# nv-tlabs/brushstroke_engine

Hardware: AMD Instinct MI355X
Metric: stylized 256x256 stroke patches/sec at batch=32 (higher is better)
Workload: dtype f16 hi x f16 hi MFMA + 2 block-scaled fp8 (e4m3) correction products per fp32 product

## Files before the change

brushstroke_engine_amd/csrc/nb_modconv_h3.hip:

```cpp
#include "nb_h3_common.h"
#include "nb_torgb.h"

static int nb_noise_src_setup(const float* noise, int64_t stride_n, int ho, int wo, const float** k_noise, long long* k_stride, NbNoiseSrcDev* k_src) {
    *k_src = NbNoiseSrcDev{nullptr, nullptr, nullptr, nullptr, nullptr, 0, 0};
    if (stride_n != NB_NOISE_IN_KERNEL) { *k_noise = noise; *k_stride = stride_n; return NB_OK; }
    const NbNoiseSrc* s = reinterpret_cast<const NbNoiseSrc*>(noise);
    if (!s || !s->noise_const_t || !s->noise_lin || !s->noise_strength || ((s->norm_pos != nullptr) == (s->positions != nullptr))) return NB_EINVAL;
    if (s->res != ho || s->res != wo || (s->positions && s->img_resolution < 2)) return NB_EINVAL;
    *k_src = NbNoiseSrcDev{s->noise_const_t, s->noise_lin, s->noise_strength, s->norm_pos, (const long long*)s->positions, s->res, s->img_resolution};
    *k_noise = nullptr; *k_stride = 0;
    return NB_OK;
}

struct H3Params {
    const _Float16* x;
    const _Float16* wts;
    const float* dcoefs;
    const float* noise;
    NbNoiseSrcDev nsrc;
    const float* bias;
    float* y;
    const float* zeros;
    long long noise_stride_n;
    int c8, nchunks, c_out, co_ld, h, w;
// ... 1741 lines not shown
                        }
                    }
                unsigned ha[2][2], hb[2][2], la[2][2], lb[2][2];
#pragma unroll
                for (int px = 0; px < 2; ++px)
#pragma unroll
                    for (int k = 0; k < 2; ++k) {
                        ha[px][k] = hi[0][px][k]; hb[px][k] = hi[1][px][k]; la[px][k] = lo[0][px][k]; lb[px][k] = lo[1][px][k];
                        nb_swap32(ha[px][k], hb[px][k]);
                        nb_swap32(la[px][k], lb[px][k]);
                    }
                const int cg = co0 / 8 + 2 * R + gs;
                const int oy = 2 * qi + lh, ox = 2 * qj;
                if (qi < H && cg * 8 < p.c_out && !(p.dbg & 1)) {
                    const size_t OHW8 = (size_t)Ho * Wo * 8;
                    _Float16* yn = p.yh2 + ((size_t)n * p.c8_next + cg) * 2 * OHW8;
                    const size_t opix8 = ((size_t)oy * Wo + ox) * 8;
#pragma unroll
                    for (int px = 0; px < 2; ++px) {
                        *reinterpret_cast<u32x4*>(yn + opix8 + px * 8) = u32x4{ha[px][0], ha[px][1], hb[px][0], hb[px][1]};
                        if constexpr (OUTM == 1) {
                            *reinterpret_cast<u32x4*>(yn + OHW8 + opix8 + px * 8) = u32x4{la[px][0], la[px][1], lb[px][0], lb[px][1]};
                        } else {
                            _Float16* lo_xl = p.yh2 + ((size_t)n * p.c8_next + (cg & ~1)) * 2 * OHW8 + OHW8 + opix8 + px * 8 + (cg & 1) * 4;
                            *reinterpret_cast<u32x2*>(lo_xl) = u32x2{la[px][0], lb[px][0]};
                            *reinterpret_cast<u32x2*>(lo_xl + 2 * OHW8) = u32x2{la[px][1], lb[px][1]};
                        }
                    }
                }
            }
        };
        constexpr int NWI = nquads * 2 / 32;
        static_assert(nquads * 2 % 32 == 0, "tile quads must fill whole waves");
        if constexpr (NWI % NW == 0) {
#pragma unroll
            for (int k = 0; k < NWI / NW; ++k) quad_item(wv + k * NW);
        } else {
            for (int wi = wv; wi < NWI; wi += NW) quad_item(wi);
        }
        if (p.tstamps) { const unsigned long long t_ = __builtin_amdgcn_s_memtime(); te_f += t_ - te0; }
    }
    const unsigned long long te_s = 0;
    NB_TSTAMP(4);
    if (p.tstamps) {
        asm volatile("s_waitcnt vmcnt(0)" ::: "memory");
        NB_TSTAMP(5);
        if (threadIdx.x == 0) p.tstamps[(size_t)(blockIdx.x + blockIdx.y * gridDim.x) * 8 + 3] = (te_w & 0x1fffff) | ((te_f & 0x1fffff) << 21) | ((te_s & 0x1fffff) << 42);
    }
}

static int g_force_tqh = -1;
extern "C" void nb_debug_set_up2_tile(int tqh) { g_force_tqh = tqh; }
bool nb_up2v_eligible(int in_fmt, int c_in, int h, int w);
int nb_up2v_launch(H3Up2Params p, int n, int in_fmt, void* stream, unsigned long long* tstamps, int tstamps_cap);
#ifndef NB_UP2V_AUTO
#define NB_UP2V_AUTO 1
#endif
static int g_force_v2 = -1;
extern "C" void nb_debug_set_up2_v2(int mode) { g_force_v2 = mode; }
static int g_force_pair = -1;
extern "C" void nb_debug_set_up2_pair(int mode) { g_force_pair = mode; }
template <int TQH, int TQW, bool F8, int OUTM, int NW, int NST>
static int nb_up2_h3_launch1(const H3Up2Params& p, int n, size_t lds, void* stream) {
    static bool attr_set = false;
    if (!attr_set) {
        (void)hipFuncSetAttribute((const void*)modconv3x3_up2_h3_kernel<F8, TQH, OUTM, TQW, NW, NST>, hipFuncAttributeMaxDynamicSharedMemorySize, (int)lds);
        attr_set = true;
    }
    dim3 grid(p.tiles_x * p.tiles_y * p.slices, n);
    hipLaunchKernelGGL((modconv3x3_up2_h3_kernel<F8, TQH, OUTM, TQW, NW, NST>), grid, dim3(NW * 64), lds, (hipStream_t)stream, p);
    NB_CHECK_LAUNCH("modconv3x3_up2_h3");
    return NB_OK;
}

template <int TQH, int TQW = 32, int NW = 8, int NST = NB_H3_STAGES>
static int nb_up2_h3_launch(H3Up2Params p, int n, int in_fmt, void* stream) {
    p.tiles_x = p.w / TQW;
    p.tiles_y = (p.h + TQH - 1) / TQH;
    p.tstamps = (g_tstamps && (long long)p.tiles_x * p.tiles_y * p.slices * n <= g_tstamps_cap) ? g_tstamps : nullptr;
    constexpr int XPL = (TQH + 3) * (TQW + 3);
    constexpr int NBLK_ = ((TQH + 2) * (TQW + 2) + 31) / 32;
    constexpr size_t lds_stage = (size_t)NST * (4 * XPL + 36 * 32) * 16;
    static_assert(NBLK_ <= 2 * NW, "two column blocks per wave at most");
    constexpr size_t lds_epi = (size_t)16 * NBLK_ * 32 * 16;
    const size_t lds = lds_stage > lds_epi ? lds_stage : lds_epi;
    const int outm = p.yh2 ? (p.out_f8 ? 2 : 1) : 0;
    if constexpr (NW == 4) {
        NB_REQUIRE(!in_fmt, "modconv3x3_up2_h3: the two-workgroups-per-CU form takes H2 operands only");
        return outm == 2 ? nb_up2_h3_launch1<TQH, TQW, false, 2, NW, NST>(p, n, lds, stream) : outm == 1 ? nb_up2_h3_launch1<TQH, TQW, false, 1, NW, NST>(p, n, lds, stream)
                                                                                               : nb_up2_h3_launch1<TQH, TQW, false, 0, NW, NST>(p, n, lds, stream);
    } else
    if (in_fmt)
        return outm == 2 ? nb_up2_h3_launch1<TQH, TQW, true, 2, NW, NST>(p, n, lds, stream) : outm == 1 ? nb_up2_h3_launch1<TQH, TQW, true, 1, NW, NST>(p, n, lds, stream)
                                                                                              : nb_up2_h3_launch1<TQH, TQW, true, 0, NW, NST>(p, n, lds, stream);
    return outm == 2 ? nb_up2_h3_launch1<TQH, TQW, false, 2, NW, NST>(p, n, lds, stream) : outm == 1 ? nb_up2_h3_launch1<TQH, TQW, false, 1, NW, NST>(p, n, lds, stream)
                                                                                           : nb_up2_h3_launch1<TQH, TQW, false, 0, NW, NST>(p, n, lds, stream);
}

enum Up2Form { UP2_BIG = 0, UP2_MID, UP2_SMALL, UP2_W16, UP2_PAIR, UP2_WIDE, UP2_V2, UP2_W8 };
static Up2Form nb_up2_h3_select(int in_fmt, int c_in, int c_out, int n, int h, int w) {
    const int tiles_x = w / 32, slices = (c_out + 31) / 32;
    if (w == 16) return UP2_W16;
    if (w == 8) return UP2_W8;
    const int force_tqh = g_force_tqh >= 0 ? g_force_tqh : 0;
    const long wgs_big = (long)n * tiles_x * ((h + NB_H3_TQH - 1) / NB_H3_TQH) * slices;
    const bool small_tiles = force_tqh ? force_tqh == NB_H3_TQH_SMALL : wgs_big < 160;
    bool mid_tiles = force_tqh == NB_H3_TQH_MID;
    if (!force_tqh && !small_tiles) {
        constexpr long ncu = 256;
        const long wgs_mid = (long)n * tiles_x * ((h + NB_H3_TQH_MID - 1) / NB_H3_TQH_MID) * slices;
        const double est_big = (double)((wgs_big + ncu - 1) / ncu) * 5.4, est_mid = (double)((wgs_mid + ncu - 1) / ncu) * 3.93;
        mid_tiles = est_mid < 0.9 * est_big;
    }
    const bool pair = !in_fmt && g_force_pair > 0;
    if (pair) return UP2_PAIR;
    const int force_v2 = g_force_v2;
    if (force_v2 != 0 && nb_up2v_eligible(in_fmt, c_in, h, w) &&
        (force_v2 > 0 ? force_tqh == 0 || force_tqh == NB_H3_TQH : (NB_UP2V_AUTO && !mid_tiles && !small_tiles && (force_tqh == 0 || force_tqh == NB_H3_TQH))))
        return UP2_V2;
    if (mid_tiles) return UP2_MID;
    return small_tiles ? UP2_SMALL : UP2_BIG;
}

static int nb_up2_h3_impl(const void* x_h2, int c_in, const void* w_h3, const float* dcoefs, const float* noise,
                          int64_t noise_stride_n, const float* bias, float* y, void* y_h2, const float* next_styles,
                          int next_stride, int c_next, int n, int h, int w, int c_out, float alpha, float gain, float clamp,
                          void* stream, int in_fmt = 0, int out_fmt = 0) {
    NB_REQUIRE(in_fmt >= 0 && in_fmt <= 3 && (out_fmt == 0 || out_fmt == 1), "modconv3x3_up2_h3: input operand format must be 0 (H2), 1 (f8), 2 (f6) or 3 (f8, hi only), "
               "output format 0 or 1 (the up=2 epilogue does not write the f6 format)");
    NB_REQUIRE(in_fmt == 0 || c_in % 16 == 0, "modconv3x3_up2_h3: the f8 / f6 operand formats need c_in %% 16 == 0 (got %d)", c_in);
    NB_REQUIRE(out_fmt == 0 || (y_h2 && c_out % 16 == 0 && c_next % 16 == 0), "modconv3x3_up2_h3: f8 output needs an H2 destination and c_out, c_next %% 16 == 0");
    NB_REQUIRE(x_h2 && w_h3 && dcoefs && bias && ((y != nullptr) != (y_h2 != nullptr)), "modconv3x3_up2_h3: null pointer");
    NB_REQUIRE(!y_h2 || (next_styles && c_out % 8 == 0 && c_next >= c_out && next_stride >= c_out && (uintptr_t)y_h2 % 16 == 0),
               "modconv3x3_up2_h3: H2 output needs the consumer's styles, c_out %% 8 == 0 and c_next >= c_out");
    NB_REQUIRE(n > 0 && n <= 65535 && c_in > 0 && c_out > 0, "modconv3x3_up2_h3: bad sizes");
    NB_REQUIRE((w % 32 == 0 || w == 16 || w == 8) && h >= 8, "modconv3x3_up2_h3: needs w %% 32 == 0, w == 16 or w == 8 (got %dx%d)", h, w);
    NB_REQUIRE(alpha >= 0.f && alpha <= 1.f && gain > 0.f, "modconv3x3_up2_h3: leaky-ReLU slope must lie in [0, 1] and the gain be positive (got %g, %g)", alpha, gain);
    NB_REQUIRE(((uintptr_t)x_h2 | (uintptr_t)w_h3 | (uintptr_t)y) % 16 == 0, "modconv3x3_up2_h3: pointers must be 16-byte aligned");
    H3Up2Params p;
    p.x = (const _Float16*)x_h2; p.wts = (const _Float16*)w_h3; p.dcoefs = dcoefs; p.noise = noise; p.bias = bias; p.y = y;
    p.zeros = nb_zero_page_ptr();
    NB_REQUIRE(p.zeros, "modconv3x3_up2_h3: could not allocate the zero page");
    p.noise_stride_n = noise_stride_n;
    NB_REQUIRE(nb_noise_src_setup(noise, noise_stride_n, 2 * h, 2 * w, &p.noise, &p.noise_stride_n, &p.nsrc) == NB_OK, "modconv3x3_up2_h3: bad NbNoiseSrc (needs the "
               "transposed constant, the grid row, the strength, exactly one of norm_pos / positions, and res = the %dx%d output)", 2 * h, 2 * w);
    p.c8 = (c_in + 7) / 8; p.nchunks = (c_in + 15) / 16; p.c_out = c_out; p.co_ld = (c_out + 63) / 64 * 64; p.h = h; p.w = w;
    p.dbg = g_nb_debug_flags; p.stagger_ticks = g_nb_stagger_ticks;
    p.alpha = alpha; p.gain = gain; p.clamp = clamp;
    p.tiles_x = w / 32; p.slices = (c_out + 31) / 32;
    p.yh2 = (_Float16*)y_h2; p.next_styles = next_styles; p.next_stride = next_stride; p.c8_next = (c_next + 7) / 8;
    p.out_f8 = out_fmt;
    const Up2Form form = nb_up2_h3_select(in_fmt, c_in, c_out, n, h, w);
    NB_REQUIRE(in_fmt != 2 || form == UP2_V2, "modconv3x3_up2_h3: f6 operands are taken by the 12-row software-pipelined kernel only (this launch: %dx%d, batch %d)", h, w, n);
    switch (form) {
        case UP2_W16: return nb_up2_h3_launch<8, 16>(p, n, in_fmt, stream);
        case UP2_W8: return nb_up2_h3_launch<8, 8>(p, n, in_fmt, stream);
        case UP2_PAIR: return nb_up2_h3_launch<NB_H3_TQH, 16, 4, 2>(p, n, in_fmt, stream);
        case UP2_V2: return nb_up2v_launch(p, n, in_fmt, stream, g_tstamps, g_tstamps_cap);
        case UP2_MID: return nb_up2_h3_launch<NB_H3_TQH_MID>(p, n, in_fmt, stream);
        case UP2_SMALL: return nb_up2_h3_launch<NB_H3_TQH_SMALL>(p, n, in_fmt, stream);
        default: return nb_up2_h3_launch<NB_H3_TQH>(p, n, in_fmt, stream);
    }
}

extern "C" int nb_modconv3x3_up2_h3_variant(int in_fmt, int c_in, int c_out, int n, int h, int w, char* buf, int buflen) {
    NB_REQUIRE(buf && buflen > 0, "modconv3x3_up2_h3_variant: bad buffer");
    NB_REQUIRE(in_fmt >= 0 && in_fmt <= 3 && n > 0 && c_in > 0 && c_out > 0 && h >= 8 && (w % 32 == 0 || w == 16 || w == 8), "modconv3x3_up2_h3_variant: bad shape");
    static const char* const names[] = {"modconv3x3_up2_h3_kernel", "modconv3x3_up2_h3_kernel", "modconv3x3_up2_h3_kernel", "modconv3x3_up2_h3_kernel",
                                        "modconv3x3_up2_h3_kernel", "modconv3x3_up2_h3_kernel", "modconv3x3_up2v_kernel", "modconv3x3_up2_h3_kernel"};
    snprintf(buf, buflen, "%s", names[nb_up2_h3_select(in_fmt, c_in, c_out, n, h, w)]);
    return NB_OK;
}

extern "C" int nb_modconv3x3_up2_h3(const void* x_h2, int c_in, const void* w_h3, const float* dcoefs, const float* noise,
                                    int64_t noise_stride_n, const float* bias, float* y, int n, int h, int w, int c_out,
                                    float alpha, float gain, float clamp, void* stream) {
    return nb_up2_h3_impl(x_h2, c_in, w_h3, dcoefs, noise, noise_stride_n, bias, y, nullptr, nullptr, 0, 0, n, h, w, c_out,
                          alpha, gain, clamp, stream);
}

extern "C" int nb_modconv3x3_up2_h3_ex(const void* x, int c_in, const void* wts, const float* dcoefs, const float* noise,
                                      int64_t noise_stride_n, const float* bias, float* y_f32, void* y_h2,
                                      const float* next_styles, int next_stride, int c_next, int in_fmt, int out_fmt, int n,
                                      int h, int w, int c_out, float alpha, float gain, float clamp, void* stream) {
    return nb_up2_h3_impl(x, c_in, wts, dcoefs, noise, noise_stride_n, bias, y_f32, y_h2, next_styles, next_stride, c_next,
                          n, h, w, c_out, alpha, gain, clamp, stream, in_fmt, out_fmt);
}

extern "C" int nb_modconv3x3_up2_h3_h2(const void* x_h2, int c_in, const void* w_h3, const float* dcoefs, const float* noise,
                                       int64_t noise_stride_n, const float* bias, const float* next_styles, int next_stride,
                                       void* y_h2, int c_next, int n, int h, int w, int c_out, float alpha, float gain,
                                       float clamp, void* stream) {
    return nb_up2_h3_impl(x_h2, c_in, w_h3, dcoefs, noise, noise_stride_n, bias, nullptr, y_h2, next_styles, next_stride,
                          c_next, n, h, w, c_out, alpha, gain, clamp, stream);
}

__global__ __launch_bounds__(256) void pack_h2_kernel(const float* __restrict__ x1, int c1, const float* __restrict__ x2, int c2,
                                                      const float* __restrict__ scale, _Float16* __restrict__ out, int c8, int hw) {
    const int n = blockIdx.z, cg = blockIdx.y;
    const int pix = blockIdx.x * 256 + threadIdx.x;
    if (pix >= hw) return;
    const int c_in = c1 + c2;
    h8 hi, lo;
#pragma unroll
    for (int j = 0; j < 8; ++j) {
        const int ch = cg * 8 + j;
        float v = 0.f;
        if (ch < c_in) {
            v = ch < c1 ? x1[((size_t)n * c1 + ch) * hw + pix] : x2[((size_t)n * c2 + (ch - c1)) * hw + pix];
            if (scale) v *= scale[(size_t)n * c_in + ch];
        }
// ... 244 lines not shown
```

brushstroke_engine_amd/csrc/nb_modconv_up2v.hip:

```cpp
#include "nb_h3_common.h"

#ifdef NB_ABL6_NOMFMA
#define NB_ABL6_F16 false
#define NB_ABL6_FP6 false
#elif defined(NB_ABL6_NOFP6)
#define NB_ABL6_F16 true
#define NB_ABL6_FP6 false
#else
#define NB_ABL6_F16 true
#define NB_ABL6_FP6 true
#endif
#ifdef NB_ABL6_NODMA
#define NB_ABL_NODMA 1
#endif
namespace {
constexpr int TQH = 12, TQW = 32, NW = 8, NT = NW * 64;
constexpr int PH = TQH + 2, PW = TQW + 2, NPOS = PH * PW;
constexpr int NBLK = (NPOS + 31) / 32, NBJ = 2;
constexpr int XR = TQH + 3, XS = TQW + 3, XPL = XR * XS;
constexpr int PP = (XPL + 63) / 64, NXP = 4 * PP;
constexpr int CO_WG = 32, WROWS = 36, WSLOTS = WROWS * CO_WG, NWP = WSLOTS / 64;
constexpr int NPC = (NXP + NWP + NW - 1) / NW;
constexpr int STAGE = 4 * XPL + WSLOTS, NST = 3;
constexpr int N4 = 2;
constexpr int KMIX = NXP / NW;
static_assert(NBLK <= NBJ * NW && KMIX * NW <= NXP && (KMIX + 1) * NW > NXP && NPC == 7, "piece list layout");
}

template <bool F8, int OUTM, bool F6 = false, bool HO = false, bool PERSIST = true>
__global__ __launch_bounds__(NT, 2) void modconv3x3_up2v_kernel(const H3Up2Params p) {
    static_assert(!F6 || F8, "the f6 form is a variant of the f8 loop");
    static_assert(!HO || (F8 && !F6), "the hi-only form is a variant of the f8 loop");
    NB_TSTAMP(0);
    if constexpr (OUTM == 2) nb_set_fp16_ovfl();
    extern __shared__ __attribute__((aligned(16))) unsigned char smem_v[];
    h8* ring = reinterpret_cast<h8*>(smem_v);

    const int tid = threadIdx.x;
    const int lane = tid & 63, wv = __builtin_amdgcn_readfirstlane(tid >> 6), lh = lane >> 5, l31 = lane & 31;
    const int H = p.h, W = p.w;
    typedef const __attribute__((address_space(4))) H3Up2Params* kparams_t;
    auto fresh_params = [&]() -> kparams_t {
        kparams_t q = (kparams_t)__builtin_amdgcn_kernarg_segment_ptr();
        asm volatile("" : "+s"(q));
        return q;
    };
    const unsigned total = (unsigned)p.items;
    int n = 0, I0 = 0, J0 = 0, co0 = 0;
    const size_t HW8 = (size_t)H * W * 8;
    auto tile_coords = [&](unsigned l) {
        kparams_t q_ = fresh_params();
        const unsigned total = (unsigned)q_->items, gx = (unsigned)q_->items_x;
        const int dbg = q_->dbg, slices = q_->slices, tiles_x = q_->tiles_x;
        unsigned b = l % gx;
        unsigned nn = l / gx;
        if (total % 8 == 0 && gridDim.x % 8 == 0 && !(dbg & (8 | 32))) {
            const unsigned q = (l & 7) * (total >> 3) + (l >> 3);
            nn = q / gx; b = q - nn * gx;
        } else if (gx % 8 == 0 && !(dbg & 8)) b = (((b & 7) + nn) & 7) * (gx >> 3) + (b >> 3);
        const int slice = b % slices; b /= slices;
        const int tile_x = b % tiles_x; const int tile_y = b / tiles_x;
        n = __builtin_amdgcn_readfirstlane((int)nn); I0 = __builtin_amdgcn_readfirstlane(tile_y * TQH);
        J0 = __builtin_amdgcn_readfirstlane(tile_x * TQW); co0 = __builtin_amdgcn_readfirstlane(slice * CO_WG);
    };
    unsigned item = __builtin_amdgcn_readfirstlane(blockIdx.x);
    tile_coords(item);
    const int nblk = wv < NBLK - (NBJ - 1) * NW ? NBJ : NBJ - 1;

    __shared__ __attribute__((aligned(16))) float s_dco[CO_WG], s_bias[CO_WG], s_nst[CO_WG];
    __shared__ __attribute__((aligned(16))) float s_noise[2 * TQH * 2 * TQW];
    auto load_channel_tables = [&]() {
        kparams_t q_ = fresh_params();
        if (tid < CO_WG) {
            const int co = co0 + tid, c_out = q_->c_out;
            const float gain = q_->gain;
            s_dco[tid] = co < c_out ? q_->dcoefs[(size_t)n * c_out + co] * gain : 0.f;
            s_bias[tid] = co < c_out ? q_->bias[co] * gain : 0.f;
            s_nst[tid] = (q_->yh2 && co < c_out) ? q_->next_styles[(size_t)n * q_->next_stride + co] : 0.f;
        }
    };
    const unsigned lds0 = (unsigned)(uintptr_t)NB_LDS_PTR(smem_v);
    const size_t wchunk = (size_t)WROWS * p.co_ld * 16;
    const char* xsrc0[KMIX];
    unsigned xstr[KMIX];
    unsigned woff[NPC - KMIX - 1];
    const char* msrc0 = nullptr;
    unsigned mstr = 0;
    int xdst_s[KMIX + 1];
    unsigned xlast_bits = 0;
#pragma unroll
    for (int k = 0; k <= KMIX; ++k) {
        int q = k * NW + wv; q = q < NXP ? q : NXP - 1;
        const int pl = q / PP, part = q - pl * PP;
        xdst_s[k] = __builtin_amdgcn_readfirstlane(pl * XPL + part * 64);
        xlast_bits |= (part == PP - 1 ? 1u : 0u) << k;
    }
    xlast_bits = __builtin_amdgcn_readfirstlane(xlast_bits);
    auto xdst = [&](int k) { return xdst_s[k]; };
    auto xmask = [&](int k) -> unsigned long long { return (xlast_bits >> k) & 1u ? (1ull << (XPL - (PP - 1) * 64)) - 1 : ~0ull; };
    auto wq = [&](int k) { int q = k * NW + wv - NXP; return __builtin_amdgcn_readfirstlane(q < 0 ? 0 : (q < NWP ? q : NWP - 1)); };
    const bool mix_isx = KMIX * NW + wv < NXP;
    const int mdst = mix_isx ? xdst(KMIX) : 4 * XPL + wq(KMIX) * 64;
    const unsigned long long mmask = mix_isx ? xmask(KMIX) : ~0ull;
    auto piece_sources = [&]() {
        kparams_t q_ = fresh_params();
        const char* zeros = reinterpret_cast<const char*>(q_->zeros);
        const int co_ld = q_->co_ld;
        const _Float16* xn = q_->x + (size_t)n * q_->c8 * 2 * HW8;
        int i0_ = I0, j0_ = J0, c0_ = co0, lane_ = lane;
        asm volatile("" : "+v"(i0_), "+v"(j0_), "+v"(c0_), "+v"(lane_));
        i0_ = __builtin_amdgcn_readfirstlane(i0_); j0_ = __builtin_amdgcn_readfirstlane(j0_); c0_ = __builtin_amdgcn_readfirstlane(c0_);
        const char* xs_mix = zeros;
        unsigned xt_mix = 0, wo_mix = 0;
#pragma unroll
        for (int k = 0; k <= KMIX; ++k) {
            int q = k * NW + wv;
            q = q < NXP ? q : NXP - 1;
            const int pl = q / PP, part = q - pl * PP;
            const int e = part * 64 + lane_;
            const char* xs_ = zeros;
            unsigned xt_ = 0;
            if (e < XPL) {
                const int r = e / XS, c = e - r * XS;
// ... 342 lines not shown
        });
        if constexpr (MODE >= 2) asm volatile("s_waitcnt vmcnt(%0) lgkmcnt(0)\n\ts_barrier" ::"n"(NPC) : "memory");
        else if constexpr (MODE == 1) asm volatile("s_waitcnt vmcnt(0) lgkmcnt(0)\n\ts_barrier" ::: "memory");
        NB_FENCE();
        group_pair(std::integral_constant<int, 0>{}, ah_n, al_n, bh2, bh3, bl23, [&](auto g_) {
            constexpr int g = decltype(g_)::value;
            if constexpr (g == 2) dma(std::integral_constant<int, 0>{});
            if constexpr (g == 5) dma(std::integral_constant<int, 1>{});
            if constexpr (MODE >= 1) {
                if constexpr (g == 0) { ah_a[0] = rA(8, 0, san); rBh(bh0, J0_{}, 0, san); }
                else if constexpr (g == 1) { ah_a[1] = rA(6, 0, san); rBh(bh1, J0_{}, 1, san); }
                else if constexpr (g == 2) { rBh(bh0, J1_{}, 0, san); rBh(bh1, J1_{}, 1, san); }
                else if constexpr (g == 3) { set_lo(al_a, rA(8, 1, san)); set_hi(al_a, rA(6, 1, san)); }
                else if constexpr (g == 4) { rBl(bl01, 0, J0_{}, 0, san); rBl(bl01, 1, J0_{}, 1, san); }
                else { rBl(bl01, 0, J1_{}, 0, san); rBl(bl01, 1, J1_{}, 1, san); }
            }
        });
        NB_FENCE();
    };
    auto kloop = [&](auto nbe) {
        constexpr int NBE = decltype(nbe)::value;
        ah_a[0] = ring[aoff + 8 * 128]; ah_a[1] = ring[aoff + 6 * 128];
        if constexpr (F6) {
            const h8* b_ = ring + a6 + (lh ? 6 : 8) * 128;
            const i32x4 q0 = __builtin_bit_cast(i32x4, b_[0]); const i32x4 q1 = __builtin_bit_cast(i32x4, b_[64]);
            al6_a = v6i{q0[0], q0[1], q0[2], q0[3], q1[0], q1[1]}; sa6_a = q1[2];
        } else if constexpr (F8) { set_lo(al_a, ring[aoff + 8 * 128 + 32]); set_hi(al_a, ring[aoff + 6 * 128 + 32]); }
        else { hl_a[0] = ring[aoff + 8 * 128 + 32]; hl_a[1] = ring[aoff + 6 * 128 + 32]; }
#pragma unroll
        for (int j = 0; j < NBE; ++j) {
            bh0[j] = ring[boff[j]]; bh1[j] = ring[boff[j] + 1];
            if constexpr (F6) {
                const h8* b_ = ring + b6[j] + lh;
                const i32x4 q0 = __builtin_bit_cast(i32x4, b_[0]); const i32x4 q1 = __builtin_bit_cast(i32x4, b_[2 * XPL]);
                bl6_01[j] = v6i{q0[0], q0[1], q0[2], q0[3], q1[0], q1[1]}; sb6_01[j] = q1[2];
            } else if constexpr (F8) { set_lo(bl01[j], ring[boff[j] + XPL]); set_hi(bl01[j], ring[boff[j] + XPL + 1]); }
            else { bl0[j] = ring[boff[j] + XPL]; bl1[j] = ring[boff[j] + XPL + 1]; }
        }
        int c = 0, s = 0;
        auto nxt = [](int s_) { return s_ == 2 ? 0 : s_ + 1; };
        for (; c + 3 < NC; ++c) {
            chunk(std::integral_constant<int, 3>{}, nbe, c, ring + s * STAGE, ring + nxt(s) * STAGE, nxt(nxt(s)) * STAGE, s * STAGE);
            s = nxt(s);
        }
        if (c + 2 < NC) { chunk(std::integral_constant<int, 2>{}, nbe, c, ring + s * STAGE, ring + nxt(s) * STAGE, nxt(nxt(s)) * STAGE, 0); s = nxt(s); ++c; }
        if (c + 1 < NC) { chunk(std::integral_constant<int, 1>{}, nbe, c, ring + s * STAGE, ring + nxt(s) * STAGE, 0, 0); s = nxt(s); ++c; }
        chunk(std::integral_constant<int, 0>{}, nbe, c, ring + s * STAGE, nullptr, 0, 0);
    };
    nb_static_for<0, NPC>([&](auto k) { issue_piece(k, 0, 0); });
  for (;;) {
#undef NB_TSTAMP
#define NB_TSTAMP(k) do { if (p.tstamps && threadIdx.x == 0) { unsigned it_ = item; asm volatile("" : "+v"(it_)); p.tstamps[(size_t)it_ * 8 + (k)] = __builtin_amdgcn_s_memrealtime(); } } while (0)
    load_channel_tables();
    {
        kparams_t q_ = fresh_params();
        const float* noise = q_->noise;
        const long long nstride = q_->noise_stride_n;
        const float gain = q_->gain;
        const NbNoiseSrcDev nsrc{q_->nsrc.const_t, q_->nsrc.lin, q_->nsrc.strength, q_->nsrc.norm_pos, q_->nsrc.positions, q_->nsrc.res, q_->nsrc.img_res};
        for (int e = tid; e < 2 * TQH * 2 * TQW; e += NT) {
            const int r = e / (2 * TQW), c = e - r * (2 * TQW);
            const int oy = 2 * I0 + r, ox = 2 * J0 + c;
            float v = (noise && oy < 2 * H) ? noise[(size_t)n * nstride + (size_t)oy * (2 * W) + ox] : 0.f;
            if (nsrc.const_t && oy < 2 * H) {
                float np0, np1, wx0, wx1, wy0, wy1;
                int sx0, sy0;
                nb_noise_np(nsrc, n, np0, np1);
                nb_noise_axis(nsrc, oy, np0, sx0, wx0, wx1);
                nb_noise_axis(nsrc, ox, np1, sy0, wy0, wy1);
                v = nb_noise_value(nsrc, nsrc.strength[0], sx0, wx0, wx1, sy0, wy0, wy1);
            }
            s_noise[e] = v * gain;
        }
    }
    if (NC > 1) nb_static_for<0, NPC>([&](auto k) { issue_piece(k, 1, STAGE); });
    if (NC > 2) nb_static_for<0, N4>([&](auto k) { issue_piece(k, 2, 2 * STAGE); });
    if (NC > 2) asm volatile("s_waitcnt vmcnt(%0)" ::"n"(NPC + N4) : "memory");
    else if (NC > 1) asm volatile("s_waitcnt vmcnt(%0)" ::"n"(NPC) : "memory");
    else asm volatile("s_waitcnt vmcnt(0)" ::: "memory");
    __builtin_amdgcn_s_barrier();
    NB_TSTAMP(1);

#pragma unroll
    for (int j = 0; j < NBJ; ++j)
#pragma unroll
        for (int ph = 0; ph < 4; ++ph)
#pragma unroll
            for (int r = 0; r < 16; ++r) acc[j][ph][r] = 0.f;
    zero_fragments();
    const unsigned t_loop0 = p.tstamps ? (unsigned)__builtin_amdgcn_s_memtime() : 0u;
    const int nvalid_blk = (min(TQH, H - I0) + 2) * PW;
    int nbe_w = 0;
#pragma unroll
    for (int j = 0; j < NBJ; ++j) nbe_w += (wv + NW * j) * 32 < nvalid_blk && j < nblk;
    if (nbe_w == 2) kloop(std::integral_constant<int, 2>{});
    else if (nbe_w == 1) kloop(std::integral_constant<int, 1>{});
    else kloop(std::integral_constant<int, 0>{});
#undef NB_FENCE
    if (p.tstamps && tid == 0) {
        unsigned it_ = item; asm volatile("" : "+v"(it_));
        unsigned long long* ts = p.tstamps + (size_t)it_ * 8;
        ts[6] = 0; ts[7] = (unsigned long long)((unsigned)__builtin_amdgcn_s_memtime() - t_loop0) << 32;
    }
    asm volatile("s_waitcnt vmcnt(0) lgkmcnt(0)" ::: "memory");
    __builtin_amdgcn_s_barrier();
#pragma unroll
    for (int k = 0; k < KMIX; ++k) { asm volatile("" : "=v"(xsrc0[k])); asm volatile("" : "=v"(xstr[k])); }
#pragma unroll
    for (int k = 0; k < NPC - KMIX - 1; ++k) asm volatile("" : "=v"(woff[k]));
    asm volatile("" : "=v"(msrc0)); asm volatile("" : "=v"(mstr));

    NB_TSTAMP(2);
    if (p.dbg & 4) { if (acc[0][0][0] == 123.456f) p.y[0] = 0.f; return; }
    const int e_n = n, e_I0 = I0, e_J0 = J0, e_co0 = co0;
    const unsigned item_next = PERSIST ? __builtin_amdgcn_readfirstlane(item + gridDim.x) : total;
    const bool has_next = item_next < total && !(p.dbg & 64);
    if (item_next < total) {
        tile_coords(item_next);
        piece_sources();
        if (has_next) {
            nb_static_for<0, KMIX>([&](auto k) { issue_piece(k, 0, 0); });
            if (mix_isx) issue_piece(std::integral_constant<int, KMIX>{}, 0, 0);
        }
    }
    int l31e = l31, lhe = lh, wve = wv;
    asm volatile("" : "+v"(l31e), "+v"(lhe), "+s"(wve));
    const int Wo = 2 * W, Ho = 2 * H;
    constexpr int nquads = TQH * TQW;
    constexpr int Y1P = NBLK * 32;
    f32x4* y4 = reinterpret_cast<f32x4*>(smem_v + (size_t)4 * XPL * 16);
    const float clampv = p.clamp >= 0.f ? p.clamp : __builtin_inff();
    unsigned long long te_w = 0, te_f = 0, te0 = 0;
#pragma unroll
    for (int R = 0; R < 2; ++R) {
        if (p.tstamps) te0 = __builtin_amdgcn_s_memtime();
        if (R) asm volatile("s_waitcnt lgkmcnt(0)\n\ts_barrier" ::: "memory");
#pragma unroll
        for (int gs = 0; gs < 2; ++gs) {
            const int r0 = (2 * R + gs) * 4;
#pragma unroll
            for (int j = 0; j < NBJ; ++j) {
                if (j >= nblk) continue;
                const int pidx = (wve + NW * j) * 32 + l31e;
#pragma unroll
                for (int ph = 0; ph < 4; ++ph) {
                    const f32x16& a_ = acc[j][ph];
                    y4[((gs * 2 + lhe) * 4 + ph) * Y1P + pidx] = f32x4{a_[r0], a_[r0 + 1], a_[r0 + 2], a_[r0 + 3]};
                }
            }
        }
        asm volatile("s_waitcnt lgkmcnt(0)\n\ts_barrier" ::: "memory");
        if (p.tstamps) { const unsigned long long t_ = __builtin_amdgcn_s_memtime(); te_w += t_ - te0; te0 = t_; }
        auto quad_item = [&](const int wi) {
            const int hq = wi * 32 + l31e;
            const int gs = hq / nquads, qd = hq - gs * nquads;
            const int ti = qd / TQW, tj = qd - ti * TQW;
            if (e_I0 + ti >= H) return;
            const int c4 = 16 * R + 8 * gs + 4 * lhe;
            const f32x4* ee = y4 + ((gs * 2 + lhe) * 4) * Y1P + ti * PW + tj;
            const f32x4* eo = ee + 1 * Y1P;
            const f32x4* oe = ee + 2 * Y1P;
            const f32x4* oo = ee + 3 * Y1P;
            auto fir4 = [](f32x4 a, f32x4 b, f32x4 c, f32x4 d) {
                f32x4 q75, q25;
                q75 = 0.75f; q25 = 0.25f;
                return __builtin_elementwise_fma(q25, d, __builtin_elementwise_fma(q75, c, __builtin_elementwise_fma(q75, b, 0.25f * a)));
            };
            f32x4 ve[2][2], vo[3][2];
#pragma unroll
            for (int c = 0; c < 3; ++c) {
                if (c < 2) {
                    const f32x4 e0 = ee[c], e1 = ee[PW + c], o0 = oe[c], o1 = oe[PW + c], o2 = oe[2 * PW + c];
                    ve[c][0] = fir4(o0, e0, o1, e1); ve[c][1] = fir4(e0, o1, e1, o2);
                }
                const f32x4 e0 = eo[c], e1 = eo[PW + c], o0 = oo[c], o1 = oo[PW + c], o2 = oo[2 * PW + c];
                vo[c][0] = fir4(o0, e0, o1, e1); vo[c][1] = fir4(e0, o1, e1, o2);
            }
            const f32x4 d4 = *reinterpret_cast<const f32x4*>(s_dco + c4), b4 = *reinterpret_cast<const f32x4*>(s_bias + c4);
            const int qi = e_I0 + ti, qj = e_J0 + tj;
            auto act4 = [&](f32x4 o, float nz) {
                f32x4 t = __builtin_elementwise_fma(o, d4, b4 + nz);
                const f32x4 ta = t * p.alpha;
#pragma unroll
                for (int i = 0; i < 4; ++i) t[i] = __builtin_amdgcn_fmed3f(__builtin_amdgcn_fmed3f(t[i], ta[i], __builtin_inff()), -clampv, clampv);
                return t;
            };
            f32x4 v[2][2];
#pragma unroll
            for (int dy = 0; dy < 2; ++dy) {
                const f32x2 nz = *reinterpret_cast<const f32x2*>(s_noise + (2 * ti + dy) * (2 * TQW) + 2 * tj);
                float nz0 = nz[0], nz1 = nz[1];
                asm volatile("v_mov_b32 %0, %0" : "+v"(nz0));
                asm volatile("v_mov_b32 %0, %0" : "+v"(nz1));
                v[dy][0] = act4(fir4(vo[0][dy], ve[0][dy], vo[1][dy], ve[1][dy]), nz0);
                v[dy][1] = act4(fir4(ve[0][dy], vo[1][dy], ve[1][dy], vo[2][dy]), nz1);
            }
            if constexpr (OUTM == 0) {
                if (qi < H && !(p.dbg & 1)) {
#pragma unroll
                    for (int i = 0; i < 4; ++i) {
                        const int co = e_co0 + c4 + i;
                        if (co < p.c_out) {
                            float* dst = p.y + ((size_t)e_n * p.c_out + co) * ((size_t)Ho * Wo) + (size_t)(2 * qi) * Wo + 2 * qj;
// ... 1 lines not shown
                            *reinterpret_cast<f32x2*>(dst + Wo) = f32x2{v[1][0][i], v[1][1][i]};
                        }
                    }
                }
            } else {
                const f32x4 ns4 = *reinterpret_cast<const f32x4*>(s_nst + c4);
                unsigned hi[2][2][2], lo[2][2][2];
#pragma unroll
                for (int dy = 0; dy < 2; ++dy)
#pragma unroll
                    for (int px = 0; px < 2; ++px) {
                        f32x4 w = v[dy][px] * ns4;
                        const h2 h01 = __builtin_convertvector(f32x2{w[0], w[1]}, h2), h23 = __builtin_convertvector(f32x2{w[2], w[3]}, h2);
                        const f32x4 xl = {nb_sub_f16(w[0], h01, false), nb_sub_f16(w[1], h01, true), nb_sub_f16(w[2], h23, false), nb_sub_f16(w[3], h23, true)};
                        hi[dy][px][0] = __builtin_bit_cast(unsigned, h01); hi[dy][px][1] = __builtin_bit_cast(unsigned, h23);
                        if constexpr (OUTM == 1) {
                            const h2 l01 = __builtin_convertvector(f32x2{xl[0], xl[1]}, h2), l23 = __builtin_convertvector(f32x2{xl[2], xl[3]}, h2);
                            lo[dy][px][0] = __builtin_bit_cast(unsigned, l01); lo[dy][px][1] = __builtin_bit_cast(unsigned, l23);
                        } else {
                            lo[dy][px][0] = nb_pk4_fp8_sat_scaled(xl[0], xl[1], xl[2], xl[3], 0x1p-9f);
                            lo[dy][px][1] = nb_pk4_fp8_sat_scaled(w[0], w[1], w[2], w[3], 4.f);
                        }
                    }
                unsigned ha[2][2], hb[2][2], la[2][2], lb[2][2];
#pragma unroll
                for (int px = 0; px < 2; ++px)
#pragma unroll
                    for (int k = 0; k < 2; ++k) {
                        ha[px][k] = hi[0][px][k]; hb[px][k] = hi[1][px][k]; la[px][k] = lo[0][px][k]; lb[px][k] = lo[1][px][k];
                        nb_swap32(ha[px][k], hb[px][k]);
                        nb_swap32(la[px][k], lb[px][k]);
                    }
                const int cg = e_co0 / 8 + 2 * R + gs;
                const int oy = 2 * qi + lhe, ox = 2 * qj;
                if (qi < H && cg * 8 < p.c_out && !(p.dbg & 1)) {
                    const size_t OHW8 = (size_t)Ho * Wo * 8;
                    _Float16* yn = p.yh2 + ((size_t)e_n * p.c8_next + cg) * 2 * OHW8;
                    const size_t opix8 = ((size_t)oy * Wo + ox) * 8;
#pragma unroll
                    for (int px = 0; px < 2; ++px) {
                        *reinterpret_cast<u32x4*>(yn + opix8 + px * 8) = u32x4{ha[px][0], ha[px][1], hb[px][0], hb[px][1]};
                        if constexpr (OUTM == 1) {
                            *reinterpret_cast<u32x4*>(yn + OHW8 + opix8 + px * 8) = u32x4{la[px][0], la[px][1], lb[px][0], lb[px][1]};
                        } else {
                            _Float16* lo_xl = p.yh2 + ((size_t)e_n * p.c8_next + (cg & ~1)) * 2 * OHW8 + OHW8 + opix8 + px * 8 + (cg & 1) * 4;
                            *reinterpret_cast<u32x2*>(lo_xl) = u32x2{la[px][0], lb[px][0]};
                            *reinterpret_cast<u32x2*>(lo_xl + 2 * OHW8) = u32x2{la[px][1], lb[px][1]};
                        }
                    }
                }
            }
        };
        constexpr int NWI = nquads * 2 / 32;
        static_assert(nquads * 2 % 32 == 0 && NWI % NW == 0, "tile quads must fill whole waves");
#pragma unroll
        for (int k = 0; k < NWI / NW; ++k) quad_item(wve + k * NW);
        if (p.tstamps) { const unsigned long long t_ = __builtin_amdgcn_s_memtime(); te_f += t_ - te0; }
    }
    NB_TSTAMP(4);
    if (p.tstamps) {
        asm volatile("s_waitcnt vmcnt(0)" ::: "memory");
        NB_TSTAMP(5);
        if (threadIdx.x == 0) { unsigned it_ = item; asm volatile("" : "+v"(it_)); p.tstamps[(size_t)it_ * 8 + 3] = (te_w & 0x1fffff) | ((te_f & 0x1fffff) << 21); }
    }
    if (item_next >= total) break;
    item = __builtin_amdgcn_readfirstlane(item_next);
    asm volatile("s_waitcnt lgkmcnt(0)\n\ts_barrier" ::: "memory");
    NB_TSTAMP(0);
    piece_sources();
    if (has_next) {
        if (!mix_isx) issue_piece(std::integral_constant<int, KMIX>{}, 0, 0);
        nb_static_for<KMIX + 1, NPC>([&](auto k) { issue_piece(k, 0, 0); });
    } else {
        nb_static_for<0, NPC>([&](auto k) { issue_piece(k, 0, 0); });
    }
  }
#undef NB_TSTAMP
#define NB_TSTAMP(k)                                                                                         \
    do {                                                                                                     \
        if (p.tstamps && threadIdx.x == 0) p.tstamps[(size_t)(blockIdx.x + blockIdx.y * gridDim.x) * 8 + (k)] = __builtin_amdgcn_s_memrealtime(); \
    } while (0)
}

extern int g_persist_wgs_per_cu;
#ifndef NB_UP2V_PERSIST_DEFAULT
#define NB_UP2V_PERSIST_DEFAULT 1
#endif
static int g_up2v_persist = -1;
extern "C" void nb_debug_set_up2v_persistent(int mode) { g_up2v_persist = mode; }

template <bool F8, int OUTM, bool F6 = false, bool HO = false, bool PERSIST = true>
static int nb_up2v_launch1(const H3Up2Params& p, int n, void* stream) {
    constexpr size_t lds_ring = (size_t)NST * STAGE * 16, lds_epi = (size_t)4 * XPL * 16 + (size_t)16 * NBLK * 32 * 16;
    constexpr size_t lds = lds_ring > lds_epi ? lds_ring : lds_epi;
    static bool attr_set = false;
    if (!attr_set) {
        (void)hipFuncSetAttribute((const void*)modconv3x3_up2v_kernel<F8, OUTM, F6, HO, PERSIST>, hipFuncAttributeMaxDynamicSharedMemorySize, (int)lds);
        attr_set = true;
    }
    static int ncu = 0;
    if (!ncu) {
        int dev = 0, v = 0;
        if (hipGetDevice(&dev) != hipSuccess || hipDeviceGetAttribute(&v, hipDeviceAttributeMultiprocessorCount, dev) != hipSuccess || v <= 0) v = 256;
        ncu = v;
    }
    const int items = p.items;
    const long want = (long)ncu * g_persist_wgs_per_cu;
    dim3 grid(PERSIST && items > want ? (unsigned)want : (unsigned)items);
    hipLaunchKernelGGL((modconv3x3_up2v_kernel<F8, OUTM, F6, HO, PERSIST>), grid, dim3(NT), lds, (hipStream_t)stream, p);
    NB_CHECK_LAUNCH("modconv3x3_up2v");
    return NB_OK;
}

bool nb_up2v_eligible(int in_fmt, int c_in, int h, int w) { return in_fmt >= 0 && in_fmt <= 3 && c_in % 16 == 0 && w % TQW == 0 && h >= 8; }

int nb_up2v_launch(H3Up2Params p, int n, int in_fmt, void* stream, unsigned long long* tstamps, int tstamps_cap) {
    NB_REQUIRE(nb_up2v_eligible(in_fmt, p.nchunks * 16, p.h, p.w) && p.co_ld % CO_WG == 0, "modconv3x3_up2v: shape not supported");
    p.tiles_x = p.w / TQW;
    p.tiles_y = (p.h + TQH - 1) / TQH;
    p.slices = (p.c_out + CO_WG - 1) / CO_WG;
    p.items_x = p.tiles_x * p.tiles_y * p.slices;
    p.items = p.items_x * n;
    p.tstamps = (tstamps && (long long)p.items <= tstamps_cap) ? tstamps : nullptr;
    const int outm = p.yh2 ? (p.out_f8 ? 2 : 1) : 0;
    const bool persist = g_up2v_persist >= 0 ? g_up2v_persist != 0 : NB_UP2V_PERSIST_DEFAULT != 0;
    auto go = [&](auto f8_, auto f6_, auto ho_) {
        constexpr bool F8_ = decltype(f8_)::value, F6_ = decltype(f6_)::value, HO_ = decltype(ho_)::value;
        if (persist) return outm == 2 ? nb_up2v_launch1<F8_, 2, F6_, HO_, true>(p, n, stream) : outm == 1 ? nb_up2v_launch1<F8_, 1, F6_, HO_, true>(p, n, stream) : nb_up2v_launch1<F8_, 0, F6_, HO_, true>(p, n, stream);
        return outm == 2 ? nb_up2v_launch1<F8_, 2, F6_, HO_, false>(p, n, stream) : outm == 1 ? nb_up2v_launch1<F8_, 1, F6_, HO_, false>(p, n, stream) : nb_up2v_launch1<F8_, 0, F6_, HO_, false>(p, n, stream);
    };
    using T = std::true_type; using F = std::false_type;
    if (in_fmt == 3) return go(T{}, F{}, T{});
    if (in_fmt == 2) return go(T{}, T{}, F{});
    if (in_fmt) return go(T{}, F{}, F{});
    return go(F{}, F{}, F{});
}
```

include/neube_hip_debug.h:

```cpp
#ifndef NEUBE_HIP_DEBUG_H
#define NEUBE_HIP_DEBUG_H

#ifdef __cplusplus
extern "C" {
#endif

void nb_debug_set_up1_rows(int nbw);

void nb_debug_set_up1_v2(int mode);
void nb_debug_set_up1_pp(int mode);

void nb_debug_set_small_waves(int waves);
void nb_debug_set_small_blocks(int blocks);

void nb_debug_set_up2_tile(int tqh);

void nb_debug_set_up2_pair(int mode);

void nb_debug_set_up2_v2(int mode);

void nb_debug_set_up1_persistent(int mode);

void nb_debug_set_up2v_persistent(int mode);

void nb_debug_set_persistent_wgs_per_cu(int k);

void nb_debug_set_enc_small(int mode);

void nb_debug_set_flags(int flags);
void nb_debug_set_stagger(int ticks);
void nb_debug_set_up1_small(int mode);
void nb_debug_set_wgrad_wgs(int wgs);
void nb_debug_set_upfirdn_generic(int on);

void nb_debug_set_timestamps(void* buf, int capacity_workgroups);
void nb_debug_set_timestamps_f32(void* buf, int capacity_workgroups);
void nb_debug_set_enc_timestamps(void* buf, int capacity_workgroups);

const float* nb_zero_page_ptr(void);

#ifdef __cplusplus
}
#endif
#endif
```

Before: 19410.

## Add 13-row tile variant for up2v conv with cost-model auto selection

Templates the up2v upsampling modconv kernel on tile height and adds a 13-row variant. That variant fills two full 32-position blocks per wave, moves the noise buffer into dynamic LDS, drops the next-item prefetch and persistence, and handles leftover quad work items. A small host-side cost model compares wave quantization and per-tile critical-path cost to pick 12 or 13 rows per shape. The aim is less padding waste and fewer tiles per image; the price is losing persistent scheduling and cross-item prefetch on the 13-row path.

```diff
diff --git a/brushstroke_engine_amd/csrc/nb_modconv_h3.hip b/brushstroke_engine_amd/csrc/nb_modconv_h3.hip
--- a/brushstroke_engine_amd/csrc/nb_modconv_h3.hip
+++ b/brushstroke_engine_amd/csrc/nb_modconv_h3.hip
@@ -1817,7 +1817,7 @@
 static int g_force_tqh = -1;
 extern "C" void nb_debug_set_up2_tile(int tqh) { g_force_tqh = tqh; }
 bool nb_up2v_eligible(int in_fmt, int c_in, int h, int w);
-int nb_up2v_launch(H3Up2Params p, int n, int in_fmt, void* stream, unsigned long long* tstamps, int tstamps_cap);
+int nb_up2v_launch(H3Up2Params p, int n, int in_fmt, void* stream, unsigned long long* tstamps, int tstamps_cap, bool auto_rows);
 #ifndef NB_UP2V_AUTO
 #define NB_UP2V_AUTO 1
 #endif
@@ -1921,7 +1921,7 @@
         case UP2_W16: return nb_up2_h3_launch<8, 16>(p, n, in_fmt, stream);
         case UP2_W8: return nb_up2_h3_launch<8, 8>(p, n, in_fmt, stream);
         case UP2_PAIR: return nb_up2_h3_launch<NB_H3_TQH, 16, 4, 2>(p, n, in_fmt, stream);
-        case UP2_V2: return nb_up2v_launch(p, n, in_fmt, stream, g_tstamps, g_tstamps_cap);
+        case UP2_V2: return nb_up2v_launch(p, n, in_fmt, stream, g_tstamps, g_tstamps_cap, g_force_v2 < 0);
         case UP2_MID: return nb_up2_h3_launch<NB_H3_TQH_MID>(p, n, in_fmt, stream);
         case UP2_SMALL: return nb_up2_h3_launch<NB_H3_TQH_SMALL>(p, n, in_fmt, stream);
         default: return nb_up2_h3_launch<NB_H3_TQH>(p, n, in_fmt, stream);
diff --git a/brushstroke_engine_amd/csrc/nb_modconv_up2v.hip b/brushstroke_engine_amd/csrc/nb_modconv_up2v.hip
--- a/brushstroke_engine_amd/csrc/nb_modconv_up2v.hip
+++ b/brushstroke_engine_amd/csrc/nb_modconv_up2v.hip
@@ -14,23 +14,38 @@
 #define NB_ABL_NODMA 1
 #endif
 namespace {
-constexpr int TQH = 12, TQW = 32, NW = 8, NT = NW * 64;
-constexpr int PH = TQH + 2, PW = TQW + 2, NPOS = PH * PW;
-constexpr int NBLK = (NPOS + 31) / 32, NBJ = 2;
-constexpr int XR = TQH + 3, XS = TQW + 3, XPL = XR * XS;
-constexpr int PP = (XPL + 63) / 64, NXP = 4 * PP;
+constexpr int TQW = 32, NW = 8, NT = NW * 64;
+constexpr int PW = TQW + 2, XS = TQW + 3, NBJ = 2;
 constexpr int CO_WG = 32, WROWS = 36, WSLOTS = WROWS * CO_WG, NWP = WSLOTS / 64;
-constexpr int NPC = (NXP + NWP + NW - 1) / NW;
-constexpr int STAGE = 4 * XPL + WSLOTS, NST = 3;
+constexpr int NST = 3;
 constexpr int N4 = 2;
-constexpr int KMIX = NXP / NW;
-static_assert(NBLK <= NBJ * NW && KMIX * NW <= NXP && (KMIX + 1) * NW > NXP && NPC == 7, "piece list layout");
+template <int TQH_>
+struct Up2vTile {
+    static constexpr int TQH = TQH_, PH = TQH + 2, NPOS = PH * PW, NBLK = (NPOS + 31) / 32;
+    static constexpr int XR = TQH + 3, XPL = XR * XS, PP = (XPL + 63) / 64, NXP = 4 * PP;
+    static constexpr int NPC = (NXP + NWP + NW - 1) / NW, STAGE = 4 * XPL + WSLOTS;
+    static constexpr int KMIX = NXP / NW;
+    static constexpr int Y1P = NBLK * 32;
+    static constexpr bool PREFETCH = TQH == 12;
+    static constexpr size_t Y4_OFF = PREFETCH ? (size_t)4 * XPL * 16 : 0;
+    static constexpr size_t NZ_OFF = Y4_OFF + (size_t)16 * Y1P * 16;
+    static constexpr size_t LDS_RING = (size_t)NST * STAGE * 16;
+    static constexpr size_t LDS_EPI = NZ_OFF + (PREFETCH ? 0 : (size_t)2 * TQH * 2 * TQW * 4);
+    static constexpr size_t LDS = LDS_RING > LDS_EPI ? LDS_RING : LDS_EPI;
+    static_assert(NBLK <= NBJ * NW && KMIX * NW <= NXP && (KMIX + 1) * NW > NXP && NPC == 7, "piece list layout");
+    static_assert(PREFETCH || NBLK == NBJ * NW, "13-row tiles: two full position blocks per wave");
+    static_assert(LDS + 400 + (PREFETCH ? (size_t)2 * TQH * 2 * TQW * 4 : 16) <= 160 * 1024, "LDS budget (dynamic + static)");
+};
 }
 
-template <bool F8, int OUTM, bool F6 = false, bool HO = false, bool PERSIST = true>
+template <bool F8, int OUTM, bool F6 = false, bool HO = false, bool PERSIST = true, int TQH_ = 12>
 __global__ __launch_bounds__(NT, 2) void modconv3x3_up2v_kernel(const H3Up2Params p) {
     static_assert(!F6 || F8, "the f6 form is a variant of the f8 loop");
     static_assert(!HO || (F8 && !F6), "the hi-only form is a variant of the f8 loop");
+    using TG = Up2vTile<TQH_>;
+    constexpr int TQH = TG::TQH, PH = TG::PH, NPOS = TG::NPOS, NBLK = TG::NBLK, XPL = TG::XPL, PP = TG::PP, NXP = TG::NXP;
+    constexpr int NPC = TG::NPC, STAGE = TG::STAGE, KMIX = TG::KMIX;
+    static_assert(PH * PW == NPOS, "");
     NB_TSTAMP(0);
     if constexpr (OUTM == 2) nb_set_fp16_ovfl();
     extern __shared__ __attribute__((aligned(16))) unsigned char smem_v[];
@@ -68,7 +83,8 @@
     const int nblk = wv < NBLK - (NBJ - 1) * NW ? NBJ : NBJ - 1;
 
     __shared__ __attribute__((aligned(16))) float s_dco[CO_WG], s_bias[CO_WG], s_nst[CO_WG];
-    __shared__ __attribute__((aligned(16))) float s_noise[2 * TQH * 2 * TQW];
+    __shared__ __attribute__((aligned(16))) float s_noise_st[TG::PREFETCH ? 2 * TQH * 2 * TQW : 4];
+    float* const s_noise = TG::PREFETCH ? s_noise_st : reinterpret_cast<float*>(smem_v + TG::NZ_OFF);
     auto load_channel_tables = [&]() {
         kparams_t q_ = fresh_params();
         if (tid < CO_WG) {
@@ -517,7 +533,7 @@
 #undef NB_TSTAMP
 #define NB_TSTAMP(k) do { if (p.tstamps && threadIdx.x == 0) { unsigned it_ = item; asm volatile("" : "+v"(it_)); p.tstamps[(size_t)it_ * 8 + (k)] = __builtin_amdgcn_s_memrealtime(); } } while (0)
     load_channel_tables();
-    {
+    auto write_noise = [&](const int tn, const int tI0, const int tJ0) {
         kparams_t q_ = fresh_params();
         const float* noise = q_->noise;
         const long long nstride = q_->noise_stride_n;
@@ -525,19 +541,20 @@
         const NbNoiseSrcDev nsrc{q_->nsrc.const_t, q_->nsrc.lin, q_->nsrc.strength, q_->nsrc.norm_pos, q_->nsrc.positions, q_->nsrc.res, q_->nsrc.img_res};
         for (int e = tid; e < 2 * TQH * 2 * TQW; e += NT) {
             const int r = e / (2 * TQW), c = e - r * (2 * TQW);
-            const int oy = 2 * I0 + r, ox = 2 * J0 + c;
-            float v = (noise && oy < 2 * H) ? noise[(size_t)n * nstride + (size_t)oy * (2 * W) + ox] : 0.f;
+            const int oy = 2 * tI0 + r, ox = 2 * tJ0 + c;
+            float v = (noise && oy < 2 * H) ? noise[(size_t)tn * nstride + (size_t)oy * (2 * W) + ox] : 0.f;
             if (nsrc.const_t && oy < 2 * H) {
                 float np0, np1, wx0, wx1, wy0, wy1;
                 int sx0, sy0;
-                nb_noise_np(nsrc, n, np0, np1);
+                nb_noise_np(nsrc, tn, np0, np1);
                 nb_noise_axis(nsrc, oy, np0, sx0, wx0, wx1);
                 nb_noise_axis(nsrc, ox, np1, sy0, wy0, wy1);
                 v = nb_noise_value(nsrc, nsrc.strength[0], sx0, wx0, wx1, sy0, wy0, wy1);
             }
             s_noise[e] = v * gain;
         }
-    }
+    };
+    if constexpr (TG::PREFETCH) write_noise(n, I0, J0);
     if (NC > 1) nb_static_for<0, NPC>([&](auto k) { issue_piece(k, 1, STAGE); });
     if (NC > 2) nb_static_for<0, N4>([&](auto k) { issue_piece(k, 2, 2 * STAGE); });
     if (NC > 2) asm volatile("s_waitcnt vmcnt(%0)" ::"n"(NPC + N4) : "memory");
@@ -579,7 +596,7 @@
     if (p.dbg & 4) { if (acc[0][0][0] == 123.456f) p.y[0] = 0.f; return; }
     const int e_n = n, e_I0 = I0, e_J0 = J0, e_co0 = co0;
     const unsigned item_next = PERSIST ? __builtin_amdgcn_readfirstlane(item + gridDim.x) : total;
-    const bool has_next = item_next < total && !(p.dbg & 64);
+    const bool has_next = TG::PREFETCH && item_next < total && !(p.dbg & 64);
     if (item_next < total) {
         tile_coords(item_next);
         piece_sources();
@@ -592,8 +609,8 @@
     asm volatile("" : "+v"(l31e), "+v"(lhe), "+s"(wve));
     const int Wo = 2 * W, Ho = 2 * H;
     constexpr int nquads = TQH * TQW;
-    constexpr int Y1P = NBLK * 32;
-    f32x4* y4 = reinterpret_cast<f32x4*>(smem_v + (size_t)4 * XPL * 16);
+    constexpr int Y1P = TG::Y1P;
+    f32x4* y4 = reinterpret_cast<f32x4*>(smem_v + TG::Y4_OFF);
     const float clampv = p.clamp >= 0.f ? p.clamp : __builtin_inff();
     unsigned long long te_w = 0, te_f = 0, te0 = 0;
 #pragma unroll
@@ -614,6 +631,7 @@
                 }
             }
         }
+        if constexpr (!TG::PREFETCH) { if (R == 0) write_noise(e_n, e_I0, e_J0); }
         asm volatile("s_waitcnt lgkmcnt(0)\n\ts_barrier" ::: "memory");
         if (p.tstamps) { const unsigned long long t_ = __builtin_amdgcn_s_memtime(); te_w += t_ - te0; te0 = t_; }
         auto quad_item = [&](const int wi) {
@@ -721,9 +739,10 @@
             }
         };
         constexpr int NWI = nquads * 2 / 32;
-        static_assert(nquads * 2 % 32 == 0 && NWI % NW == 0, "tile quads must fill whole waves");
+        static_assert(nquads * 2 % 32 == 0 && NWI % NW <= NW / 2, "tile quads must fill whole waves");
 #pragma unroll
         for (int k = 0; k < NWI / NW; ++k) quad_item(wve + k * NW);
+        if constexpr (NWI % NW != 0) { if (wve < NWI % NW) quad_item(NWI / NW * NW + wve); }
         if (p.tstamps) { const unsigned long long t_ = __builtin_amdgcn_s_memtime(); te_f += t_ - te0; }
     }
     NB_TSTAMP(4);
@@ -758,45 +777,77 @@
 static int g_up2v_persist = -1;
 extern "C" void nb_debug_set_up2v_persistent(int mode) { g_up2v_persist = mode; }
 
-template <bool F8, int OUTM, bool F6 = false, bool HO = false, bool PERSIST = true>
-static int nb_up2v_launch1(const H3Up2Params& p, int n, void* stream) {
-    constexpr size_t lds_ring = (size_t)NST * STAGE * 16, lds_epi = (size_t)4 * XPL * 16 + (size_t)16 * NBLK * 32 * 16;
-    constexpr size_t lds = lds_ring > lds_epi ? lds_ring : lds_epi;
-    static bool attr_set = false;
-    if (!attr_set) {
-        (void)hipFuncSetAttribute((const void*)modconv3x3_up2v_kernel<F8, OUTM, F6, HO, PERSIST>, hipFuncAttributeMaxDynamicSharedMemorySize, (int)lds);
-        attr_set = true;
-    }
-    static int ncu = 0;
+static long up2v_ncu() {
+    static long ncu = 0;
     if (!ncu) {
         int dev = 0, v = 0;
         if (hipGetDevice(&dev) != hipSuccess || hipDeviceGetAttribute(&v, hipDeviceAttributeMultiprocessorCount, dev) != hipSuccess || v <= 0) v = 256;
         ncu = v;
     }
+    return ncu;
+}
+
+template <bool F8, int OUTM, bool F6 = false, bool HO = false, bool PERSIST = true, int TQH = 12>
+static int nb_up2v_launch1(const H3Up2Params& p, int n, void* stream) {
+    constexpr size_t lds = Up2vTile<TQH>::LDS;
+    static bool attr_set = false;
+    if (!attr_set) {
+        (void)hipFuncSetAttribute((const void*)modconv3x3_up2v_kernel<F8, OUTM, F6, HO, PERSIST, TQH>, hipFuncAttributeMaxDynamicSharedMemorySize, (int)lds);
+        attr_set = true;
+    }
     const int items = p.items;
-    const long want = (long)ncu * g_persist_wgs_per_cu;
+    const long want = up2v_ncu() * g_persist_wgs_per_cu;
     dim3 grid(PERSIST && items > want ? (unsigned)want : (unsigned)items);
-    hipLaunchKernelGGL((modconv3x3_up2v_kernel<F8, OUTM, F6, HO, PERSIST>), grid, dim3(NT), lds, (hipStream_t)stream, p);
+    hipLaunchKernelGGL((modconv3x3_up2v_kernel<F8, OUTM, F6, HO, PERSIST, TQH>), grid, dim3(NT), lds, (hipStream_t)stream, p);
     NB_CHECK_LAUNCH("modconv3x3_up2v");
     return NB_OK;
 }
 
 bool nb_up2v_eligible(int in_fmt, int c_in, int h, int w) { return in_fmt >= 0 && in_fmt <= 3 && c_in % 16 == 0 && w % TQW == 0 && h >= 8; }
 
-int nb_up2v_launch(H3Up2Params p, int n, int in_fmt, void* stream, unsigned long long* tstamps, int tstamps_cap) {
+static int g_up2v_rows = 0;
+extern "C" void nb_debug_set_up2v_rows(int rows) { g_up2v_rows = rows; }
+
+static int nb_up2v_rows(int nchunks, int n, int h, int w, int slices, long ncu) {
+    auto est = [&](int tqh, double rest) {
+        const int tiles_y = (h + tqh - 1) / tqh;
+        double sum = 0.0;
+        for (int ty = 0; ty < tiles_y; ++ty) {
+            const int rows = h - ty * tqh < tqh ? h - ty * tqh : tqh;
+            const int blocks = ((rows + 2) * PW + 31) / 32, crit = (blocks + 3) / 4;
+            sum += 0.44 * nchunks * crit + rest;
+        }
+        const long items = (long)n * (w / TQW) * tiles_y * slices;
+        return (double)((items + ncu - 1) / ncu) * (sum / tiles_y);
+    };
+    return est(13, 19.7) < 0.98 * est(12, 18.5) ? 13 : 12;
+}
+
+extern "C" int nb_debug_up2v_auto_rows(int c_in, int c_out, int n, int h, int w) {
+    return nb_up2v_rows((c_in + 15) / 16, n, h, w, (c_out + CO_WG - 1) / CO_WG, up2v_ncu());
+}
+
+int nb_up2v_launch(H3Up2Params p, int n, int in_fmt, void* stream, unsigned long long* tstamps, int tstamps_cap, bool auto_rows) {
     NB_REQUIRE(nb_up2v_eligible(in_fmt, p.nchunks * 16, p.h, p.w) && p.co_ld % CO_WG == 0, "modconv3x3_up2v: shape not supported");
+    p.slices = (p.c_out + CO_WG - 1) / CO_WG;
+    const int rows = g_up2v_rows == 12 || g_up2v_rows == 13 ? g_up2v_rows : auto_rows ? nb_up2v_rows(p.nchunks, n, p.h, p.w, p.slices, up2v_ncu()) : 12;
     p.tiles_x = p.w / TQW;
-    p.tiles_y = (p.h + TQH - 1) / TQH;
-    p.slices = (p.c_out + CO_WG - 1) / CO_WG;
+    p.tiles_y = (p.h + rows - 1) / rows;
     p.items_x = p.tiles_x * p.tiles_y * p.slices;
     p.items = p.items_x * n;
     p.tstamps = (tstamps && (long long)p.items <= tstamps_cap) ? tstamps : nullptr;
     const int outm = p.yh2 ? (p.out_f8 ? 2 : 1) : 0;
-    const bool persist = g_up2v_persist >= 0 ? g_up2v_persist != 0 : NB_UP2V_PERSIST_DEFAULT != 0;
+    const bool persist = rows == 12 && (g_up2v_persist >= 0 ? g_up2v_persist != 0 : NB_UP2V_PERSIST_DEFAULT != 0);
+    auto go1 = [&](auto f8_, auto f6_, auto ho_, auto rows_) {
+        constexpr bool F8_ = decltype(f8_)::value, F6_ = decltype(f6_)::value, HO_ = decltype(ho_)::value;
+        constexpr int R_ = decltype(rows_)::value;
+        if constexpr (R_ == 12) {
+            if (persist) return outm == 2 ? nb_up2v_launch1<F8_, 2, F6_, HO_, true, R_>(p, n, stream) : outm == 1 ? nb_up2v_launch1<F8_, 1, F6_, HO_, true, R_>(p, n, stream) : nb_up2v_launch1<F8_, 0, F6_, HO_, true, R_>(p, n, stream);
+        }
+        return outm == 2 ? nb_up2v_launch1<F8_, 2, F6_, HO_, false, R_>(p, n, stream) : outm == 1 ? nb_up2v_launch1<F8_, 1, F6_, HO_, false, R_>(p, n, stream) : nb_up2v_launch1<F8_, 0, F6_, HO_, false, R_>(p, n, stream);
+    };
     auto go = [&](auto f8_, auto f6_, auto ho_) {
-        constexpr bool F8_ = decltype(f8_)::value, F6_ = decltype(f6_)::value, HO_ = decltype(ho_)::value;
-        if (persist) return outm == 2 ? nb_up2v_launch1<F8_, 2, F6_, HO_, true>(p, n, stream) : outm == 1 ? nb_up2v_launch1<F8_, 1, F6_, HO_, true>(p, n, stream) : nb_up2v_launch1<F8_, 0, F6_, HO_, true>(p, n, stream);
-        return outm == 2 ? nb_up2v_launch1<F8_, 2, F6_, HO_, false>(p, n, stream) : outm == 1 ? nb_up2v_launch1<F8_, 1, F6_, HO_, false>(p, n, stream) : nb_up2v_launch1<F8_, 0, F6_, HO_, false>(p, n, stream);
+        return rows == 13 ? go1(f8_, f6_, ho_, std::integral_constant<int, 13>{}) : go1(f8_, f6_, ho_, std::integral_constant<int, 12>{});
     };
     using T = std::true_type; using F = std::false_type;
     if (in_fmt == 3) return go(T{}, F{}, T{});
diff --git a/include/neube_hip_debug.h b/include/neube_hip_debug.h
--- a/include/neube_hip_debug.h
+++ b/include/neube_hip_debug.h
@@ -23,6 +23,9 @@
 
 void nb_debug_set_up2v_persistent(int mode);
 
+void nb_debug_set_up2v_rows(int rows);
+int nb_debug_up2v_auto_rows(int c_in, int c_out, int n, int h, int w);
+
 void nb_debug_set_persistent_wgs_per_cu(int k);
 
 void nb_debug_set_enc_small(int mode);
```

New measurement: 19780, median of 6. 1.02x the previous value.
